# spacemeshos/go-spacemesh

Measured on NVIDIA H100. Metric: POST labels/sec (scrypt N=8192 init), higher is better.
Workload: dtype u32

## Files before the change

go-spacemesh_b200/csrc/capi.cu:

```cuda
#include <algorithm>
#include <chrono>
#include <cstring>
#include <string>
#include <vector>

#include "../../include/b200post.h"
#include "../../include/b200post_verify.h"
#include "../../include/post_compat.h"
#include "engine.h"
#include "host_hash.h"
#include "randomx_engine.h"

using namespace b200post;

namespace {

bool valid_n(uint64_t n) { return n >= 2 && n <= (1ull << 20) && (n & (n - 1)) == 0; }

void fill_nonce(b200post_vrf_nonce *dst, const VrfResult &r) {
    if (!dst) return;
    memset(dst, 0, sizeof *dst);
    dst->found = r.found ? 1 : 0;
    if (r.found) { dst->index = r.index; memcpy(dst->label32, r.label32, 32); }
}
// ... 9 lines not shown
    if (int rc = device_engine(provider, &e)) return rc;
    VrfResult vr;
    const int rc = e->labels_range(commitment, n, start, count, out_host, out_dev, vrf_difficulty, &vr, cancel);
    if (rc == B200POST_OK) fill_nonce(nonce, vr);
    return rc;
}

}

extern "C" {

int b200post_providers(b200post_provider *out, int max) {
    const int n = device_count();
    for (int i = 0; i < n && out && i < max; i++) {
        cudaDeviceProp p;
        if (cudaGetDeviceProperties(&p, i) != cudaSuccess) continue;
        memset(&out[i], 0, sizeof out[i]);
        out[i].id = (uint32_t)i;
        out[i].device_class = B200POST_DEVICE_CLASS_GPU;
        strncpy(out[i].model, p.name, sizeof(out[i].model) - 1);
        out[i].hbm_bytes = p.totalGlobalMem;
        out[i].sm_count = (uint32_t)p.multiProcessorCount;
        out[i].cc_major = (uint32_t)p.major; out[i].cc_minor = (uint32_t)p.minor;
    }
    return n;
}

const char *b200post_last_error(void) { return last_error(); }

int b200post_set_option(const char *key, int64_t value) {
    if (!key) return B200POST_ERR_INVALID_ARGUMENT;
    Options &o = options();
    const std::string k(key);
    if (k == "romix_variant" && value >= 0 && value <= 4) { o.romix_variant = value; return B200POST_OK; }
    if (k == "rotate_mask" && value >= 0 && value <= 1 && romix_mask_supported((int)value)) { o.rotate_mask = value; return B200POST_OK; }
    if (k == "tpb" && (value == 64 || value == 128 || value == 256 || value == 512)) { o.tpb = value; return B200POST_OK; }
    if (k == "dr_unroll" && (value == 1 || value == 4)) { o.dr_unroll = value; return B200POST_OK; }
    if (k == "ctas_per_sm" && value >= 0 && value <= 32) { o.ctas_per_sm = value; return B200POST_OK; }
    if (k == "max_scratch_mib" && value >= 0) { o.max_scratch_mib = value; return B200POST_OK; }
    if (k == "speculate_next" && (value == 0 || value == 1)) { o.speculate_next = value; return B200POST_OK; }
    if (k == "debug_corrupt_next_batch" && (value == 0 || value == 1)) { o.debug_corrupt_next_batch = value; return B200POST_OK; }
    if (k == "debug_corrupt_check_all" && (value == 0 || value == 1)) { o.debug_corrupt_check_all = value; return B200POST_OK; }
    if (k == "lowlat_max_labels" && value >= 0 && value <= (1 << 20)) { o.lowlat_max_labels = value; return B200POST_OK; }
    if (k == "rx_vm_mode" && value >= 0 && value <= 3) { o.rx_vm_mode = value; return B200POST_OK; }
    if (k == "rx_vms_per_sm" && value >= 0 && value <= 4096) { o.rx_vms_per_sm = value; return B200POST_OK; }
    if (k == "debug_skip_phase" && value >= 0 && value <= 3) { o.debug_skip_phase = value; return B200POST_OK; }
    set_error("unknown option or value out of range: " + k);
    return B200POST_ERR_INVALID_ARGUMENT;
}

int64_t b200post_get_option(const char *key) {
    if (!key) return -1;
    Options &o = options();
    const std::string k(key);
    if (k == "romix_variant") return o.romix_variant;
    if (k == "rotate_mask") return o.rotate_mask;
    if (k == "tpb") return o.tpb;
    if (k == "dr_unroll") return o.dr_unroll;
    if (k == "ctas_per_sm") return o.ctas_per_sm;
    if (k == "max_scratch_mib") return o.max_scratch_mib;
    if (k == "speculate_next") return o.speculate_next;
    if (k == "rx_vms_per_sm") return o.rx_vms_per_sm;
    if (k == "rx_vm_mode") return o.rx_vm_mode;
    if (k == "lowlat_max_labels") return o.lowlat_max_labels;
    if (k == "debug_skip_phase") return o.debug_skip_phase;
    return -1;
}
// ... 230 lines not shown
```

go-spacemesh_b200/csrc/engine.cu:

```cuda
#include "engine.h"

#include <algorithm>
#include <cstdio>
#include <cstdlib>
#include <cstring>
#include <map>
#include <memory>
#include <thread>
#include <vector>

#include "../../include/b200post.h"
#include "../../include/b200post_setup.h"
#include "metrics.h"

namespace b200post {

Options &options() { static Options o; return o; }
std::atomic<uint64_t> g_launches{0};

static thread_local std::string t_error;
void set_error(const std::string &msg) { t_error = msg; }
const char *last_error() { return t_error.c_str(); }
int fail(int rc, const std::string &msg) { set_error(msg); return rc; }

// ... 7 lines not shown
    if (copy_stream_.get()) cudaStreamSynchronize(copy_stream_.get());
}

int DeviceEngine::Layer::allocate(uint32_t slots) {
    CUDA_TRY(X.resize((size_t)slots * 8));
    CUDA_TRY(d_out.resize((size_t)slots * 16));
    CUDA_TRY(h_out.resize((size_t)slots * 16));
    CUDA_TRY(d_commit.resize((size_t)slots * 32));
    CUDA_TRY(h_commit.resize((size_t)slots * 32));
    CUDA_TRY(d_idx.resize(slots));
    CUDA_TRY(h_idx.resize(slots));
    CUDA_TRY(d_cidx.resize(slots));
    CUDA_TRY(h_cidx.resize(slots));
    CUDA_TRY(d_exp.resize((size_t)slots * 16));
    CUDA_TRY(h_exp.resize((size_t)slots * 16));
    CUDA_TRY(d_bits.resize(slots / 32));
    CUDA_TRY(d_cnt.resize(1));
    CUDA_TRY(h_cnt.resize(1));
    CUDA_TRY(ev_done.create(cudaEventDisableTiming));
    CUDA_TRY(ev_k3.create(cudaEventDisableTiming));
    CUDA_TRY(ev_in.create(cudaEventDisableTiming));
    CUDA_TRY(ev_exp.create(cudaEventDisableTiming));
    CUDA_TRY(ev_k2a.create(cudaEventDefault));
    CUDA_TRY(ev_k2b.create(cudaEventDefault));
    in_pending = k2_pending = false;
    pend.live = false;
    return B200POST_OK;
}

int DeviceEngine::ensure(uint64_t N, uint64_t want_slots) {
    Options &o = options();
    const int variant = (int)o.romix_variant.load(), mw = (int)o.rotate_mask.load();
    int tpb = (int)o.tpb.load();
    if (variant != ROMIX_PIPELINED && tpb != 128 && tpb != 256) tpb = 128;
    const int dr = (int)o.dr_unroll.load();
    if (!stream_.get()) {
        CUDA_TRY(stream_.create(cudaStreamNonBlocking));
        CUDA_TRY(copy_stream_.create(cudaStreamNonBlocking));
        for (Event &e : ev_call_) CUDA_TRY(e.create(cudaEventDefault));
        CUDA_TRY(d_diff_.resize(8));
        CUDA_TRY(d_range_commit_.resize(8));
        CUDA_TRY(d_running_.resize(1));
        CUDA_TRY(h_running_.resize(1));
    }
    const size_t pads = variant == ROMIX_PIPELINED ? 2 : 1;
    const size_t per_slot = 128 * (size_t)N * pads;
    size_t free_b = 0, total_b = 0;
    CUDA_TRY(cudaMemGetInfo(&free_b, &total_b));
    size_t budget = (size_t)((double)(free_b + v_bytes_) * 0.95);
    const int64_t cap_mib = o.max_scratch_mib.load();
    if (cap_mib > 0) budget = std::min(budget, (size_t)cap_mib << 20);
    const size_t sms = (size_t)prop_.multiProcessorCount;
    const int64_t want_ctas = o.ctas_per_sm.load();
    auto ctas_for = [&](int t) {
        int c = romix_max_ctas_per_sm(variant, mw, t, dr);
        if (want_ctas > 0) c = std::min<int>(c, (int)want_ctas);
        while (c > 0 && per_slot * (size_t)t * sms * (size_t)c > budget) c--;
        return c;
    };
    if (romix_max_ctas_per_sm(variant, mw, tpb, dr) <= 0) { set_error("romix kernel cannot be resident (unsupported variant / mask / tpb combination)"); return B200POST_ERR_INVALID_ARGUMENT; }
    int ctas = ctas_for(tpb);
    if (variant == ROMIX_PIPELINED) {
        for (int t = tpb / 2; t >= 64; t /= 2) {
            const int c = ctas_for(t);
            if ((uint64_t)c * t > (uint64_t)ctas * tpb) { ctas = c; tpb = t; }
        }
    }
    if (ctas == 0) ctas = 1;
    variant_ = variant; mw_ = mw; tpb_ = tpb; dr_unroll_ = dr;
    uint64_t wave = (uint64_t)sms * (uint64_t)ctas * (uint64_t)tpb;
    if (per_slot * wave > budget) {
        wave = budget / per_slot / 32 * 32;
        if (wave == 0) { set_error("not enough HBM for one warp of ROMix scratch"); return B200POST_ERR_OUT_OF_MEMORY; }
    }
    if (wave != wave_slots_) spec_.valid = false;
    wave_slots_ = (uint32_t)wave;

    const uint32_t need = (uint32_t)std::min<uint64_t>(wave, round_up((uint32_t)std::min<uint64_t>(want_slots, wave), 32));
    const size_t need_v = per_slot * (size_t)need;
    if (need_v > v_bytes_ || 128 * (size_t)N * 32 > v_align_) {
        CUDA_TRY(cudaStreamSynchronize(stream_.get()));
        spec_.valid = false;
        V_raw_.reset(); V_ = nullptr; v_bytes_ = 0;
        const size_t align = std::min<size_t>(128 * (size_t)N * 32, (size_t)1 << 32);
        CUDA_TRY(V_raw_.resize(need_v + align));
        V_ = reinterpret_cast<uint4 *>(((uintptr_t)V_raw_.get() + align - 1) / align * align);
        v_bytes_ = need_v;
        v_align_ = align;
    }
    if (need > alloc_slots_) {
        CUDA_TRY(cudaStreamSynchronize(stream_.get()));
        spec_.valid = false;
        alloc_slots_ = 0;
        for (Layer &l : layer_) { int rc = l.allocate(need); if (rc) return rc; }
        CUDA_TRY(d_cta_cand_.resize(pbkdf2_final_ctas(need)));
        alloc_slots_ = need;
    }
    return B200POST_OK;
}

void DeviceEngine::harvest(int buf) {
    Layer &l = layer_[buf];
    if (!l.k2_pending) return;
    float ms = 0;
    if (cudaEventSynchronize(l.ev_k2b.get()) == cudaSuccess &&
        cudaEventElapsedTime(&ms, l.ev_k2a.get(), l.ev_k2b.get()) == cudaSuccess) {
        romix_ms_ += ms; romix_launches_++; romix_labels_ += l.k2_labels;
    }
    l.k2_pending = false;
}

int DeviceEngine::retire(const Job &job, int b) {
    Layer &l = layer_[b];
    if (!l.pend.live) return B200POST_OK;
    CUDA_TRY(cudaEventSynchronize(l.ev_done.get()));
    if (job.out_host) memcpy(job.out_host + l.pend.off * 16, l.h_out.get(), (size_t)l.pend.n * 16);
    if (job.cmp && *l.h_cnt.get()) {
        std::vector<uint32_t> bits(round_up(l.pend.n, 32) / 32);
        CUDA_TRY(cudaMemcpy(bits.data(), l.d_bits.get(), bits.size() * 4, cudaMemcpyDeviceToHost));
        job.cmp->mismatches += *l.h_cnt.get();
        for (size_t w = 0; w < bits.size() && job.cmp->first.size() < CompareResult::kMaxReported; w++)
            for (uint32_t v = bits[w]; v && job.cmp->first.size() < CompareResult::kMaxReported; v &= v - 1)
                job.cmp->first.push_back(l.pend.off + 32 * w + (uint64_t)__builtin_ctz(v));
    }
    l.pend.live = false;
    return B200POST_OK;
}

int DeviceEngine::stage_layer(const Job &job, uint64_t layer, int b, uint32_t n_valid, LabelJob *lj) {
    Layer &l = layer_[b];
    const uint64_t off = layer * (uint64_t)std::min<uint64_t>(wave_slots_, alloc_slots_);
    *lj = LabelJob{d_range_commit_.get(), 0, nullptr, job.start + off, n_valid, nullptr};
    if (job.gather) {
        if (l.in_pending) { CUDA_TRY(cudaEventSynchronize(l.ev_in.get())); l.in_pending = false; }
        memcpy(l.h_idx.get(), job.indices + off, (size_t)n_valid * 8);
        CUDA_TRY(cudaMemcpyAsync(l.d_idx.get(), l.h_idx.get(), (size_t)n_valid * 8, cudaMemcpyHostToDevice, stream_.get()));
        lj->indices = l.d_idx.get();
        lj->start = 0;
        if (job.commit_index) {
            memcpy(l.h_cidx.get(), job.commit_index + off, (size_t)n_valid * 4);
            CUDA_TRY(cudaMemcpyAsync(l.d_cidx.get(), l.h_cidx.get(), (size_t)n_valid * 4, cudaMemcpyHostToDevice, stream_.get()));
            lj->commit = reinterpret_cast<const uint32_t *>(d_ctab_.get());
            lj->commit_index = l.d_cidx.get();
        } else if (job.commitments) {
            memcpy(l.h_commit.get(), job.commitments + off * 32, (size_t)n_valid * 32);
            CUDA_TRY(cudaMemcpyAsync(l.d_commit.get(), l.h_commit.get(), (size_t)n_valid * 32, cudaMemcpyHostToDevice, stream_.get()));
            lj->commit = reinterpret_cast<const uint32_t *>(l.d_commit.get());
            lj->commit_stride = 8;
        }
        CUDA_TRY(cudaEventRecord(l.ev_in.get(), stream_.get()));
        l.in_pending = true;
    }
    CUDA_TRY(launch_pbkdf2_expand(*lj, l.X.get(), alloc_slots_, round_up(n_valid, 32), stream_.get()));
    g_launches += 1;
    return B200POST_OK;
}

int DeviceEngine::finish_layer(const Job &job, uint64_t layer, int b, uint32_t n_valid, const LabelJob &lj) {
    Layer &l = layer_[b];
    const uint64_t off = layer * (uint64_t)std::min<uint64_t>(wave_slots_, alloc_slots_);
    const uint32_t n_slots = round_up(n_valid, 32);
    if (job.expect_host) {
        memcpy(l.h_exp.get(), job.expect_host + off * 16, (size_t)n_valid * 16);
        CUDA_TRY(cudaMemcpyAsync(l.d_exp.get(), l.h_exp.get(), (size_t)n_valid * 16, cudaMemcpyHostToDevice, copy_stream_.get()));
        CUDA_TRY(cudaEventRecord(l.ev_exp.get(), copy_stream_.get()));
        CUDA_TRY(cudaStreamWaitEvent(stream_.get(), l.ev_exp.get(), 0));
        CUDA_TRY(cudaMemsetAsync(l.d_cnt.get(), 0, 4, stream_.get()));
        CUDA_TRY(launch_pbkdf2_final_compare(lj, l.X.get(), alloc_slots_, n_slots, l.d_exp.get(), l.d_bits.get(), l.d_cnt.get(),
                                           job.d_diff, d_cta_cand_.get(), stream_.get()));
    } else if (job.out_hi_dev) {
        CUDA_TRY(launch_pbkdf2_final_wide(lj, l.X.get(), alloc_slots_, n_slots, job.out_dev + off * 16, job.out_hi_dev + off * 16,
                                          stream_.get()));
    } else {
        uint8_t *d_out = job.out_dev ? job.out_dev + off * 16 : l.d_out.get();
        CUDA_TRY(launch_pbkdf2_final(lj, l.X.get(), alloc_slots_, n_slots, d_out, job.d_diff, d_cta_cand_.get(), stream_.get()));
    }
    g_launches += 1;
    if (job.d_diff) {
        CUDA_TRY(launch_vrf_merge(d_cta_cand_.get(), pbkdf2_final_ctas(n_slots), d_running_.get(), stream_.get()));
        g_launches += 1;
    }
    if (job.out_host || job.expect_host) {
        CUDA_TRY(cudaEventRecord(l.ev_k3.get(), stream_.get()));
        CUDA_TRY(cudaStreamWaitEvent(copy_stream_.get(), l.ev_k3.get(), 0));
        if (job.expect_host)
            CUDA_TRY(cudaMemcpyAsync(l.h_cnt.get(), l.d_cnt.get(), 4, cudaMemcpyDeviceToHost, copy_stream_.get()));
        else
            CUDA_TRY(cudaMemcpyAsync(l.h_out.get(), l.d_out.get(), (size_t)n_valid * 16, cudaMemcpyDeviceToHost, copy_stream_.get()));
        CUDA_TRY(cudaEventRecord(l.ev_done.get(), copy_stream_.get()));
    } else {
        CUDA_TRY(cudaEventRecord(l.ev_done.get(), stream_.get()));
    }
    l.pend = Layer::Pending{off, n_valid, true};
    return B200POST_OK;
}

int DeviceEngine::run_job(const Job &job) {
    const uint64_t S = std::min<uint64_t>(wave_slots_, alloc_slots_);
    const uint64_t M = (job.total + S - 1) / S;
    int rc_ = B200POST_OK, status = B200POST_OK;
    auto layer_count = [&](uint64_t m) { return (uint32_t)std::min<uint64_t>(S, job.total - m * S); };
    cudaStream_t st = stream_.get();

    const int64_t lowlat_max = options().lowlat_max_labels.load();
    const bool lowlat = variant_ == ROMIX_PIPELINED && M == 1 && lowlat_max > 0 && job.total <= (uint64_t)lowlat_max &&
                        job.total <= (uint64_t)prop_.multiProcessorCount * 4 * 32;
    if (lowlat || variant_ != ROMIX_PIPELINED) {
        spec_.valid = false;
        for (uint64_t m = 0; m < M; m++) {
            if (job.cancel && *job.cancel) { status = B200POST_ERR_CANCELLED; break; }
            const int b = (int)(m & 1);
            Layer &l = layer_[b];
            if ((rc_ = retire(job, b))) return rc_;
            harvest(b);
            const uint32_t n_valid = layer_count(m);
            LabelJob lj;
            if ((rc_ = stage_layer(job, m, b, n_valid, &lj))) return rc_;
            RomixParams rp;
            rp.V = V_; rp.X = l.X.get(); rp.x_stride = alloc_slots_; rp.N = (uint32_t)job.N;
            CUDA_TRY(cudaEventRecord(l.ev_k2a.get(), st));
            if (lowlat) {
                rp.n_slots = n_valid; rp.flags = 0;
                CUDA_TRY(launch_romix_lowlat(mw_, rp, romix_lowlat_warps(n_valid, prop_.multiProcessorCount), st));
            } else {
                rp.n_slots = round_up(n_valid, 32); rp.flags = (uint32_t)options().debug_skip_phase.load();
                CUDA_TRY(launch_romix(variant_, mw_, tpb_, rp, st));
            }
            CUDA_TRY(cudaEventRecord(l.ev_k2b.get(), st));
            l.k2_pending = true; l.k2_labels = n_valid;
            g_launches += 1;
            if ((rc_ = finish_layer(job, m, b, n_valid, lj))) return rc_;
        }
    } else {
        const bool resume = !job.gather && spec_.valid && spec_.N == job.N && spec_.next_start == job.start &&
                            !memcmp(spec_.commitment, cur_commitment_, 32);
        const int poff = resume ? spec_.parity : 0;
        spec_.valid = false;
        const bool speculate = !job.gather && options().speculate_next.load() != 0 && M >= 4 && job.start + job.total + S > job.start + job.total;
        auto par = [&](uint64_t m) { return (int)((m + (uint64_t)poff) & 1); };
        LabelJob lj[2];
        uint32_t nv[2] = {0, 0};
        bool spec_filled = false;
        for (uint64_t m = 0; m <= M; m++) {
            if (m < M && job.cancel && *job.cancel) { status = B200POST_ERR_CANCELLED; break; }
            const int b = par(m);
            Layer &l = layer_[b];
            harvest(b);
            bool fill = false;
            uint32_t n_fill = 0;
            if (m < M) {
                nv[b] = layer_count(m);
                if (m == 0 && resume) {
                    lj[b] = LabelJob{d_range_commit_.get(), 0, nullptr, job.start, nv[b], nullptr};
                } else {
                    if ((rc_ = stage_layer(job, m, b, nv[b], &lj[b]))) return rc_;
                    fill = true; n_fill = round_up(nv[b], 32);
                }
            } else if (speculate && status == B200POST_OK) {
// ... 291 lines not shown
```

go-spacemesh_b200/csrc/engine.h:

```cpp
#pragma once
#include <cuda_runtime.h>

#include <atomic>
#include <cstdint>
#include <functional>
#include <mutex>
#include <string>
#include <vector>

#include "label_kernels.cuh"
#include "cuda_util.h"

namespace b200post {

struct Options {
    std::atomic<int64_t> romix_variant{ROMIX_PIPELINED};
    std::atomic<int64_t> rotate_mask{0};
    std::atomic<int64_t> tpb{512};
    std::atomic<int64_t> dr_unroll{4};
    std::atomic<int64_t> ctas_per_sm{0};
    std::atomic<int64_t> max_scratch_mib{0};
    std::atomic<int64_t> speculate_next{1};
    std::atomic<int64_t> lowlat_max_labels{4096};
    std::atomic<int64_t> rx_vms_per_sm{0};
    std::atomic<int64_t> rx_vm_mode{1};
    std::atomic<int64_t> debug_corrupt_next_batch{0};
    std::atomic<int64_t> debug_corrupt_check_all{0};
    std::atomic<int64_t> debug_skip_phase{0};
};
Options &options();

extern std::atomic<uint64_t> g_launches;

struct VrfResult { bool found = false; uint64_t index = 0; uint8_t label32[32] = {0}; };
struct CompareResult {
    static constexpr size_t kMaxReported = 64;
    uint64_t mismatches = 0;
    std::vector<uint64_t> first;
};

void set_error(const std::string &msg);
const char *last_error();
int fail(int rc, const std::string &msg);

class DeviceEngine {
public:
    explicit DeviceEngine(int device);
    ~DeviceEngine();
    DeviceEngine(const DeviceEngine &) = delete;
// ... 45 lines not shown
        DeviceBuffer<uint32_t> d_bits, d_cnt;
        PinnedBuffer<uint32_t> h_cnt;
        Event ev_done;
        Event ev_k3;
        Event ev_in;
        Event ev_exp;
        Event ev_k2a, ev_k2b;
        bool in_pending = false, k2_pending = false;
        double k2_labels = 0;
        struct Pending { uint64_t off; uint32_t n; bool live; } pend{0, 0, false};
        int allocate(uint32_t slots);
    };
    int call(Job &job, const std::function<int()> &setup);
    int ensure(uint64_t N, uint64_t want_slots);
    int run_job(const Job &job);
    int range_call(Job &job, const uint8_t commitment[32], const uint8_t *vrf_difficulty);
    int upload_commitment(const uint8_t commitment[32]);
    int stage_layer(const Job &job, uint64_t layer, int b, uint32_t n_valid, LabelJob *lj);
    int finish_layer(const Job &job, uint64_t layer, int b, uint32_t n_valid, const LabelJob &lj);
    int retire(const Job &job, int buf);
    void harvest(int buf);
    void quiesce();

    int dev_;
    cudaDeviceProp prop_{};
    std::mutex mu_;
    Stream stream_;
    Stream copy_stream_;
    DeviceBuffer<uint8_t> V_raw_;
    uint4 *V_ = nullptr;
    size_t v_bytes_ = 0, v_align_ = 0;
    uint32_t alloc_slots_ = 0;
    uint32_t wave_slots_ = 0;
    Layer layer_[2];
    DeviceBuffer<uint32_t> d_range_commit_;
    DeviceBuffer<uint8_t> d_ctab_;
    DeviceBuffer<uint32_t> d_diff_;
    DeviceBuffer<VrfCandidate> d_cta_cand_, d_running_;
    PinnedBuffer<VrfCandidate> h_running_;
    Event ev_call_[2];
    double last_call_ms_ = 0;
    Event ev_timer_[2];
    double romix_ms_ = 0, romix_labels_ = 0;
    uint64_t romix_launches_ = 0;
    struct Speculation {
        bool valid = false;
        uint8_t commitment[32] = {0};
        uint64_t N = 0, next_start = 0;
        int parity = 0;
    } spec_;
    uint8_t cur_commitment_[32] = {0};
    int variant_ = ROMIX_PIPELINED, mw_ = 0, tpb_ = 512, dr_unroll_ = 4;
};

DeviceEngine *engine_for(uint32_t provider);
int device_engine(uint32_t provider, DeviceEngine **e = nullptr);
int device_engines(const uint32_t *providers, int n, std::vector<DeviceEngine *> *out = nullptr);
int device_count();
int provider_devices(int64_t provider_id, std::vector<uint32_t> *devs);
void shutdown_all();

int fan_out(size_t parts, const std::function<int(size_t)> &part);

int label32_at(DeviceEngine *e, const uint8_t commitment[32], uint64_t N, uint64_t index, uint8_t out[32]);

}
// ... 1 lines not shown
```

go-spacemesh_b200/csrc/label_kernels.cu:

```cuda
#include "label_kernels.cuh"

namespace b200post {

__device__ __forceinline__ uint32_t smem_u32(const void *p) { return (uint32_t)__cvta_generic_to_shared(p); }

__device__ __forceinline__ uint4 ld_stream(const uint4 *p) {
    uint4 v;
    asm volatile("ld.global.cs.v4.u32 {%0,%1,%2,%3}, [%4];" : "=r"(v.x), "=r"(v.y), "=r"(v.z), "=r"(v.w) : "l"(p));
    return v;
}
__device__ __forceinline__ void st_stream(uint4 *p, const uint4 &v) {
    asm volatile("st.global.cs.v4.u32 [%0], {%1,%2,%3,%4};" ::"l"(p), "r"(v.x), "r"(v.y), "r"(v.z), "r"(v.w) : "memory");
}
__device__ __forceinline__ void cp_async16(uint32_t dst_smem, const void *src) {
    asm volatile("cp.async.cg.shared.global [%0], [%1], 16;" ::"r"(dst_smem), "l"(src) : "memory");
}
template <int IMM>
__device__ __forceinline__ void cp_async16_lohi(uint32_t dst_smem, uint32_t lo, uint32_t hi) {
    asm volatile("{\n\t.reg .b64 a;\n\tmov.b64 a, {%1, %2};\n\tcp.async.cg.shared.global [%0], [a+%3], 16;\n\t}"
                 ::"r"(dst_smem), "r"(lo), "r"(hi), "n"(IMM) : "memory");
}
template <int IMM>
__device__ __forceinline__ void st_stream_lohi(uint32_t lo, uint32_t hi, const uint4 &v) {
    asm volatile("{\n\t.reg .b64 a;\n\tmov.b64 a, {%0, %1};\n\tst.global.cs.v4.u32 [a+%2], {%3,%4,%5,%6};\n\t}"
// ... 272 lines not shown
    };

    if (do_mix) mix_prefetch();
    for (uint32_t i = 0; i < N; i++) {
        if (do_fill) {
            fill_store();
            blockmix_r1<MW, DR_UNROLL>(lo_f, hi_f);
        }
        if (do_mix) {
            cp_async_wait_all();
            __syncwarp();
            uint32_t vlo[16], vhi[16];
#pragma unroll
            for (int k = 0; k < 8; k++) set_chunk(vlo, vhi, k, lds128(own_m + ((k ^ swz) << 4)));
            __syncwarp();
            blockmix_r1_xor<MW, DR_UNROLL>(lo_m, hi_m, vlo, vhi);
            if (i + 1 < N) mix_prefetch();
        }
    }
#undef MIX_PREFETCH_K
#undef FILL_STORE_K
    if (do_fill) {
#pragma unroll
        for (int k = 0; k < 8; k++) p.Xfill[(size_t)k * p.x_stride + slot] = ROW_CHUNK(lo_f, hi_f, k);
    }
    if (do_mix) {
#pragma unroll
        for (int k = 0; k < 8; k++) p.Xmix[(size_t)k * p.x_stride + slot] = ROW_CHUNK(lo_m, hi_m, k);
    }
    if (p.cta_trace && threadIdx.x == 0) {
        unsigned long long t;
        asm volatile("mov.u64 %0, %%globaltimer;" : "=l"(t));
        p.cta_trace[3 * (size_t)blockIdx.x + 1] = t;
    }
}

constexpr int FINAL_TPB = 128;

__device__ __forceinline__ void warp_argmin(uint32_t (&best)[8], uint64_t &best_i, uint32_t &has) {
#pragma unroll
    for (int off = 16; off > 0; off >>= 1) {
        uint32_t o[8];
#pragma unroll
        for (int k = 0; k < 8; k++) o[k] = __shfl_xor_sync(0xffffffffu, best[k], off);
        const uint64_t oi = __shfl_xor_sync(0xffffffffu, best_i, off);
        const uint32_t oh = __shfl_xor_sync(0xffffffffu, has, off);
        const bool take = oh && (!has || cand_less(o, oi, best, best_i));
        if (take) {
#pragma unroll
            for (int k = 0; k < 8; k++) best[k] = o[k];
            best_i = oi; has = 1;
        }
    }
}

__device__ __forceinline__ void cta_vrf_candidate(bool valid, const uint32_t (&lab)[8], uint64_t index,
                                                  const uint32_t *__restrict__ vrf_be, VrfCandidate *warp_best,
                                                  VrfCandidate *__restrict__ cta_cand) {
    uint32_t diff[8];
#pragma unroll
    for (int k = 0; k < 8; k++) diff[k] = vrf_be[k];
    const bool cand = valid && cand_less(lab, 0, diff, 0);
    if (!__syncthreads_or(cand)) {
        if (threadIdx.x == 0) cta_cand[blockIdx.x].found = 0;
        return;
    }
// ... 181 lines not shown
cudaError_t launch_pbkdf2_final_compare(const LabelJob &job, const uint4 *X, uint32_t x_stride, uint32_t n_slots,
                                        const uint8_t *expect16, uint32_t *mismatch_bits, uint32_t *mismatch_count,
                                        const uint32_t *vrf_difficulty_be, VrfCandidate *cta_cand, cudaStream_t s) {
    if (n_slots == 0) return cudaSuccess;
    pbkdf2_final_compare_kernel<<<pbkdf2_final_ctas(n_slots), FINAL_TPB, 0, s>>>(job, X, x_stride, n_slots, expect16, mismatch_bits,
                                                                                 mismatch_count, vrf_difficulty_be, cta_cand);
    return cudaGetLastError();
}

cudaError_t launch_pbkdf2_final(const LabelJob &job, const uint4 *X, uint32_t x_stride, uint32_t n_slots, uint8_t *out16,
                                const uint32_t *vrf_difficulty_be, VrfCandidate *cta_cand, cudaStream_t s) {
    if (n_slots == 0) return cudaSuccess;
    pbkdf2_final_kernel<<<pbkdf2_final_ctas(n_slots), FINAL_TPB, 0, s>>>(job, X, x_stride, n_slots, out16,
                                                                         vrf_difficulty_be, cta_cand);
    return cudaGetLastError();
}

cudaError_t launch_pbkdf2_final_wide(const LabelJob &job, const uint4 *X, uint32_t x_stride, uint32_t n_slots, uint8_t *out16,
                                     uint8_t *out_hi16, cudaStream_t s) {
    if (n_slots == 0) return cudaSuccess;
    pbkdf2_final_wide_kernel<<<pbkdf2_final_ctas(n_slots), FINAL_TPB, 0, s>>>(job, X, x_stride, n_slots, out16, out_hi16);
    return cudaGetLastError();
}

cudaError_t launch_vrf_merge(const VrfCandidate *cta_cand, uint32_t n_cta, VrfCandidate *running, cudaStream_t s) {
    vrf_merge_kernel<<<1, 256, 0, s>>>(cta_cand, n_cta, running);
    return cudaGetLastError();
}

size_t romix_smem_bytes(int variant, int tpb) {
    const size_t warps = (size_t)tpb / 32;
    if (variant == ROMIX_COALESCED) return warps * 4096;
    if (variant == ROMIX_BULK) return warps * 8192 + warps * 8;
    if (variant == ROMIX_PIPELINED) return warps * 8192;
    return 0;
}

const char *romix_variant_name(int variant) {
    switch (variant) {
        case ROMIX_DIRECT: return "direct";
        case ROMIX_COALESCED: return "coalesced";
        case ROMIX_BULK: return "bulk";
        case ROMIX_NOMEM: return "nomem";
        case ROMIX_PIPELINED: return "pipelined";
    }
    return "?";
}

typedef void (*romix_fn)(const RomixParams);
typedef void (*pipe_fn)(const PipeParams);

#define B200POST_MW_LIST(X) X(0) X(1)

template <int VARIANT, int MW>
static romix_fn pick_tpb(int tpb) {
    switch (tpb) {
        case 128: return romix_kernel<VARIANT, MW, 128>;
        case 256: return romix_kernel<VARIANT, MW, 256>;
    }
    return nullptr;
}
template <int VARIANT>
static romix_fn pick_mw(int mw, int tpb) {
    switch (mw) {
#define X(m) case m: return pick_tpb<VARIANT, m>(tpb);
        B200POST_MW_LIST(X)
#undef X
    }
    return nullptr;
}
static romix_fn pick(int variant, int mw, int tpb) {
    switch (variant) {
        case ROMIX_DIRECT: return pick_mw<ROMIX_DIRECT>(mw, tpb);
        case ROMIX_COALESCED: return pick_mw<ROMIX_COALESCED>(mw, tpb);
        case ROMIX_BULK: return pick_mw<ROMIX_BULK>(mw, tpb);
        case ROMIX_NOMEM: return pick_mw<ROMIX_NOMEM>(mw, tpb);
    }
    return nullptr;
}
template <int MW>
static pipe_fn pick_pipe_tpb(int tpb, int dr_unroll) {
    if (dr_unroll == 4) {
        switch (tpb) {
            case 64: return romix_pipe_kernel<MW, 64, 4>;
            case 128: return romix_pipe_kernel<MW, 128, 4>;
            case 256: return romix_pipe_kernel<MW, 256, 4>;
            case 512: return romix_pipe_kernel<MW, 512, 4>;
        }
    } else {
        switch (tpb) {
            case 64: return romix_pipe_kernel<MW, 64, 1>;
            case 128: return romix_pipe_kernel<MW, 128, 1>;
            case 256: return romix_pipe_kernel<MW, 256, 1>;
            case 512: return romix_pipe_kernel<MW, 512, 1>;
        }
    }
    return nullptr;
}
static pipe_fn pick_pipe(int mw, int tpb, int dr_unroll) {
    switch (mw) {
#define X(m) case m: return pick_pipe_tpb<m>(tpb, dr_unroll);
        B200POST_MW_LIST(X)
#undef X
    }
    return nullptr;
}

bool romix_mask_supported(int mw) {
    switch (mw) {
#define X(m) case m: return true;
        B200POST_MW_LIST(X)
#undef X
    }
    return false;
}

int romix_max_ctas_per_sm(int variant, int rot_mask, int tpb, int dr_unroll) {
    const size_t smem = romix_smem_bytes(variant, tpb);
    int n = 0;
    if (variant == ROMIX_PIPELINED) {
        pipe_fn fn = pick_pipe(rot_mask, tpb, dr_unroll);
        if (!fn) return 0;
        if (smem > 48 * 1024) cudaFuncSetAttribute(fn, cudaFuncAttributeMaxDynamicSharedMemorySize, (int)smem);
        if (cudaOccupancyMaxActiveBlocksPerMultiprocessor(&n, fn, tpb, smem) != cudaSuccess) return 0;
        return n;
    }
    romix_fn fn = pick(variant, rot_mask, tpb);
    if (!fn) return 0;
    if (smem > 48 * 1024) cudaFuncSetAttribute(fn, cudaFuncAttributeMaxDynamicSharedMemorySize, (int)smem);
    if (cudaOccupancyMaxActiveBlocksPerMultiprocessor(&n, fn, tpb, smem) != cudaSuccess) return 0;
    return n;
}

cudaError_t launch_romix(int variant, int rot_mask, int tpb, const RomixParams &p, cudaStream_t s) {
    if (p.n_slots == 0) return cudaSuccess;
    romix_fn fn = pick(variant, rot_mask, tpb);
    if (!fn) return cudaErrorInvalidValue;
    const size_t smem = romix_smem_bytes(variant, tpb);
    if (smem > 48 * 1024) {
        cudaError_t e = cudaFuncSetAttribute(fn, cudaFuncAttributeMaxDynamicSharedMemorySize, (int)smem);
        if (e != cudaSuccess) return e;
    }
    fn<<<(p.n_slots + tpb - 1) / tpb, tpb, smem, s>>>(p);
    return cudaGetLastError();
}

uint32_t romix_lowlat_warps(uint32_t n_slots, int sm_count) {
    const uint32_t full = (uint32_t)sm_count * 4;
    return n_slots < full ? (n_slots ? n_slots : 1) : full;
}
cudaError_t launch_romix_lowlat(int rot_mask, const RomixParams &p, uint32_t n_warps, cudaStream_t s) {
    if (p.n_slots == 0) return cudaSuccess;
    if (n_warps == 0 || (uint64_t)n_warps * 32 < p.n_slots) return cudaErrorInvalidValue;
    if (rot_mask == 1) romix_lowlat_kernel<1><<<n_warps, 32, 0, s>>>(p, n_warps);
    else romix_lowlat_kernel<0><<<n_warps, 32, 0, s>>>(p, n_warps);
    return cudaGetLastError();
}

cudaError_t launch_romix_pipe(int rot_mask, int tpb, int dr_unroll, const PipeParams &p, cudaStream_t s) {
    const uint32_t n = p.n_fill > p.n_mix ? p.n_fill : p.n_mix;
    if (n == 0) return cudaSuccess;
    pipe_fn fn = pick_pipe(rot_mask, tpb, dr_unroll);
    if (!fn) return cudaErrorInvalidValue;
    const size_t smem = romix_smem_bytes(ROMIX_PIPELINED, tpb);
    if (smem > 48 * 1024) {
        cudaError_t e = cudaFuncSetAttribute(fn, cudaFuncAttributeMaxDynamicSharedMemorySize, (int)smem);
        if (e != cudaSuccess) return e;
    }
    fn<<<(n + tpb - 1) / tpb, tpb, smem, s>>>(p);
    return cudaGetLastError();
}

}
```

go-spacemesh_b200/csrc/label_kernels.cuh:

```cuda
#pragma once
#include <cuda_runtime.h>
#include <cstdint>

#include "post_device.cuh"

namespace b200post {

enum RomixVariant : int {
    ROMIX_DIRECT = 0,
    ROMIX_COALESCED = 1,
    ROMIX_BULK = 2,
    ROMIX_NOMEM = 3,
    ROMIX_PIPELINED = 4,
};

struct RomixParams {
    uint4 *V;
    uint4 *X;
    uint32_t x_stride;
    uint32_t N;
    uint32_t n_slots;
    uint32_t flags;
};

struct PipeParams {
    uint4 *V;
    uint4 *Xfill;
    uint4 *Xmix;
    uint32_t x_stride;
    uint32_t N;
    uint32_t n_fill, n_mix;
    uint32_t fill_parity;
    unsigned long long *cta_trace;
};

struct LabelJob {
    const uint32_t *commit;
    uint32_t commit_stride;
    const uint64_t *indices;
    uint64_t start;
    uint32_t n_valid;
    const uint32_t *commit_index;
};

struct VrfCandidate {
    uint32_t label_be[8];
    uint64_t index;
    uint32_t found, pad;
};

cudaError_t launch_pbkdf2_expand(const LabelJob &job, uint4 *X, uint32_t x_stride, uint32_t n_slots, cudaStream_t s);
cudaError_t launch_romix(int variant, int rot_mask, int tpb, const RomixParams &p, cudaStream_t s);
cudaError_t launch_romix_pipe(int rot_mask, int tpb, int dr_unroll, const PipeParams &p, cudaStream_t s);
uint32_t romix_lowlat_warps(uint32_t n_slots, int sm_count);
cudaError_t launch_romix_lowlat(int rot_mask, const RomixParams &p, uint32_t n_warps, cudaStream_t s);
// ... 19 lines not shown
```

go-spacemesh_b200/csrc/post_device.cuh:

```cuda
#pragma once
#include <cstdint>

#if defined(__CUDACC__)
#define PD_HD __host__ __device__ __forceinline__
#define PD_D __device__ __forceinline__
#else
#define PD_HD inline
#define PD_D inline
#endif

namespace b200post {

PD_HD uint32_t rotl(uint32_t x, int k) {
#if defined(__CUDA_ARCH__)
    return __funnelshift_l(x, x, k);
#else
    return (x << k) | (x >> (32 - k));
#endif
}
PD_HD uint32_t bswap32(uint32_t x) {
#if defined(__CUDA_ARCH__)
    return __byte_perm(x, 0, 0x0123);
#else
    return (x >> 24) | ((x >> 8) & 0xff00u) | ((x << 8) & 0xff0000u) | (x << 24);
// ... 47 lines not shown

template <int ROT, int DR_UNROLL = 4>
PD_HD void blockmix_r1(uint32_t (&lo)[16], uint32_t (&hi)[16]) {
#pragma unroll
    for (int i = 0; i < 16; i++) lo[i] ^= hi[i];
    chacha20_8<ROT, DR_UNROLL>(lo);
#pragma unroll
    for (int i = 0; i < 16; i++) hi[i] ^= lo[i];
    chacha20_8<ROT, DR_UNROLL>(hi);
}
template <int ROT, int DR_UNROLL = 4>
PD_HD void blockmix_r1_xor(uint32_t (&lo)[16], uint32_t (&hi)[16], const uint32_t (&vlo)[16],
                           const uint32_t (&vhi)[16]) {
#pragma unroll
    for (int i = 0; i < 16; i++) { hi[i] ^= vhi[i]; lo[i] = lo[i] ^ vlo[i] ^ hi[i]; }
    chacha20_8<ROT, DR_UNROLL>(lo);
#pragma unroll
    for (int i = 0; i < 16; i++) hi[i] ^= lo[i];
    chacha20_8<ROT, DR_UNROLL>(hi);
}

template <int ROT, int DR_UNROLL>
PD_HD void blockmix_r1_dual(uint32_t (&lo_f)[16], uint32_t (&hi_f)[16], uint32_t (&lo_m)[16], uint32_t (&hi_m)[16],
                            const uint32_t (&vlo)[16], const uint32_t (&vhi)[16]) {
#pragma unroll
    for (int i = 0; i < 16; i++) {
        lo_f[i] ^= hi_f[i];
        hi_m[i] ^= vhi[i]; lo_m[i] = lo_m[i] ^ vlo[i] ^ hi_m[i];
    }
    chacha20_8_x2<ROT, DR_UNROLL>(lo_f, lo_m);
#pragma unroll
    for (int i = 0; i < 16; i++) { hi_f[i] ^= lo_f[i]; hi_m[i] ^= lo_m[i]; }
    chacha20_8_x2<ROT, DR_UNROLL>(hi_f, hi_m);
}

#define PD_KECCAK_RC_TABLE \
    0x0000000000000001ull, 0x0000000000008082ull, 0x800000000000808aull, 0x8000000080008000ull, 0x000000000000808bull, \
    0x0000000080000001ull, 0x8000000080008081ull, 0x8000000000008009ull, 0x000000000000008aull, 0x0000000000000088ull, \
    0x0000000080008009ull, 0x000000008000000aull, 0x000000008000808bull, 0x800000000000008bull, 0x8000000000008089ull, \
    0x8000000000008003ull, 0x8000000000008002ull, 0x8000000000000080ull, 0x000000000000800aull, 0x800000008000000aull, \
    0x8000000080008081ull, 0x8000000000008080ull, 0x0000000080000001ull, 0x8000000080008008ull
static const uint64_t h_KeccakRC[24] = {PD_KECCAK_RC_TABLE};
#if defined(__CUDACC__)
static __device__ __constant__ uint64_t c_KeccakRC[24] = {PD_KECCAK_RC_TABLE};
#endif
PD_HD uint64_t keccak_rc(int i) {
#if defined(__CUDA_ARCH__)
    return c_KeccakRC[i];
#else
    return h_KeccakRC[i];
#endif
}
PD_HD uint64_t rotl64(uint64_t x, int k) { return (x << k) | (x >> (64 - k)); }

PD_HD void keccak_f1600(uint64_t (&s)[25]) {
#pragma unroll 1
    for (int round = 0; round < 24; round++) {
        const uint64_t c0 = s[0] ^ s[5] ^ s[10] ^ s[15] ^ s[20], c1 = s[1] ^ s[6] ^ s[11] ^ s[16] ^ s[21],
                       c2 = s[2] ^ s[7] ^ s[12] ^ s[17] ^ s[22], c3 = s[3] ^ s[8] ^ s[13] ^ s[18] ^ s[23],
                       c4 = s[4] ^ s[9] ^ s[14] ^ s[19] ^ s[24];
        const uint64_t d0 = c4 ^ rotl64(c1, 1), d1 = c0 ^ rotl64(c2, 1), d2 = c1 ^ rotl64(c3, 1),
                       d3 = c2 ^ rotl64(c4, 1), d4 = c3 ^ rotl64(c0, 1);
#pragma unroll
        for (int y = 0; y < 25; y += 5) { s[y] ^= d0; s[y + 1] ^= d1; s[y + 2] ^= d2; s[y + 3] ^= d3; s[y + 4] ^= d4; }
        uint64_t t = s[1], u;
#define PD_RP(j, r) u = s[j]; s[j] = rotl64(t, r); t = u;
// ... 133 lines not shown
```

Before: 1.235 million.

## Add phased ROMix kernel processing two labels per thread as default

Adds a new ROMix variant in which each thread carries two independent scrypt states (slot and slot+T). Their fill-phase blockmixes are interleaved, and in the read phase each state's random-row cp.async fetch overlaps the other state's mix. The intent is to hide HBM latency with instruction-level parallelism instead of warp-level occupancy. The engine now sizes a layer at twice the wave, sets the new variant as the default, and drops the speculative pipelined path. The cost is doubled registers per thread, which may reduce occupancy.

```diff
diff --git a/go-spacemesh_b200/csrc/capi.cu b/go-spacemesh_b200/csrc/capi.cu
--- a/go-spacemesh_b200/csrc/capi.cu
+++ b/go-spacemesh_b200/csrc/capi.cu
@@ -65,7 +65,7 @@
     if (!key) return B200POST_ERR_INVALID_ARGUMENT;
     Options &o = options();
     const std::string k(key);
-    if (k == "romix_variant" && value >= 0 && value <= 4) { o.romix_variant = value; return B200POST_OK; }
+    if (k == "romix_variant" && value >= 0 && value <= 5) { o.romix_variant = value; return B200POST_OK; }
     if (k == "rotate_mask" && value >= 0 && value <= 1 && romix_mask_supported((int)value)) { o.rotate_mask = value; return B200POST_OK; }
     if (k == "tpb" && (value == 64 || value == 128 || value == 256 || value == 512)) { o.tpb = value; return B200POST_OK; }
     if (k == "dr_unroll" && (value == 1 || value == 4)) { o.dr_unroll = value; return B200POST_OK; }
diff --git a/go-spacemesh_b200/csrc/engine.cu b/go-spacemesh_b200/csrc/engine.cu
--- a/go-spacemesh_b200/csrc/engine.cu
+++ b/go-spacemesh_b200/csrc/engine.cu
@@ -63,7 +63,8 @@
     Options &o = options();
     const int variant = (int)o.romix_variant.load(), mw = (int)o.rotate_mask.load();
     int tpb = (int)o.tpb.load();
-    if (variant != ROMIX_PIPELINED && tpb != 128 && tpb != 256) tpb = 128;
+    const bool two_pads = variant == ROMIX_PIPELINED || variant == ROMIX_PHASED;
+    if (!two_pads && tpb != 128 && tpb != 256) tpb = 128;
     const int dr = (int)o.dr_unroll.load();
     if (!stream_.get()) {
         CUDA_TRY(stream_.create(cudaStreamNonBlocking));
@@ -74,7 +75,7 @@
         CUDA_TRY(d_running_.resize(1));
         CUDA_TRY(h_running_.resize(1));
     }
-    const size_t pads = variant == ROMIX_PIPELINED ? 2 : 1;
+    const size_t pads = two_pads ? 2 : 1;
     const size_t per_slot = 128 * (size_t)N * pads;
     size_t free_b = 0, total_b = 0;
     CUDA_TRY(cudaMemGetInfo(&free_b, &total_b));
@@ -91,7 +92,7 @@
     };
     if (romix_max_ctas_per_sm(variant, mw, tpb, dr) <= 0) { set_error("romix kernel cannot be resident (unsupported variant / mask / tpb combination)"); return B200POST_ERR_INVALID_ARGUMENT; }
     int ctas = ctas_for(tpb);
-    if (variant == ROMIX_PIPELINED) {
+    if (two_pads) {
         for (int t = tpb / 2; t >= 64; t /= 2) {
             const int c = ctas_for(t);
             if ((uint64_t)c * t > (uint64_t)ctas * tpb) { ctas = c; tpb = t; }
@@ -106,9 +107,11 @@
     }
     if (wave != wave_slots_) spec_.valid = false;
     wave_slots_ = (uint32_t)wave;
-
-    const uint32_t need = (uint32_t)std::min<uint64_t>(wave, round_up((uint32_t)std::min<uint64_t>(want_slots, wave), 32));
-    const size_t need_v = per_slot * (size_t)need;
+    const uint64_t layer = variant == ROMIX_PHASED ? 2 * wave : wave;
+    layer_labels_ = (uint32_t)layer;
+
+    const uint32_t need = (uint32_t)std::min<uint64_t>(layer, round_up((uint32_t)std::min<uint64_t>(want_slots, layer), 32));
+    const size_t need_v = per_slot * (size_t)std::min<uint64_t>(need, wave);
     if (need_v > v_bytes_ || 128 * (size_t)N * 32 > v_align_) {
         CUDA_TRY(cudaStreamSynchronize(stream_.get()));
         spec_.valid = false;
@@ -160,7 +163,7 @@
 
 int DeviceEngine::stage_layer(const Job &job, uint64_t layer, int b, uint32_t n_valid, LabelJob *lj) {
     Layer &l = layer_[b];
-    const uint64_t off = layer * (uint64_t)std::min<uint64_t>(wave_slots_, alloc_slots_);
+    const uint64_t off = layer * (uint64_t)std::min<uint64_t>(layer_labels_, alloc_slots_);
     *lj = LabelJob{d_range_commit_.get(), 0, nullptr, job.start + off, n_valid, nullptr};
     if (job.gather) {
         if (l.in_pending) { CUDA_TRY(cudaEventSynchronize(l.ev_in.get())); l.in_pending = false; }
@@ -189,7 +192,7 @@
 
 int DeviceEngine::finish_layer(const Job &job, uint64_t layer, int b, uint32_t n_valid, const LabelJob &lj) {
     Layer &l = layer_[b];
-    const uint64_t off = layer * (uint64_t)std::min<uint64_t>(wave_slots_, alloc_slots_);
+    const uint64_t off = layer * (uint64_t)std::min<uint64_t>(layer_labels_, alloc_slots_);
     const uint32_t n_slots = round_up(n_valid, 32);
     if (job.expect_host) {
         memcpy(l.h_exp.get(), job.expect_host + off * 16, (size_t)n_valid * 16);
@@ -227,14 +230,14 @@
 }
 
 int DeviceEngine::run_job(const Job &job) {
-    const uint64_t S = std::min<uint64_t>(wave_slots_, alloc_slots_);
+    const uint64_t S = std::min<uint64_t>(layer_labels_, alloc_slots_);
     const uint64_t M = (job.total + S - 1) / S;
     int rc_ = B200POST_OK, status = B200POST_OK;
     auto layer_count = [&](uint64_t m) { return (uint32_t)std::min<uint64_t>(S, job.total - m * S); };
     cudaStream_t st = stream_.get();
 
     const int64_t lowlat_max = options().lowlat_max_labels.load();
-    const bool lowlat = variant_ == ROMIX_PIPELINED && M == 1 && lowlat_max > 0 && job.total <= (uint64_t)lowlat_max &&
+    const bool lowlat = (variant_ == ROMIX_PIPELINED || variant_ == ROMIX_PHASED) && M == 1 && lowlat_max > 0 && job.total <= (uint64_t)lowlat_max &&
                         job.total <= (uint64_t)prop_.multiProcessorCount * 4 * 32;
     if (lowlat || variant_ != ROMIX_PIPELINED) {
         spec_.valid = false;
@@ -255,6 +258,7 @@
                 CUDA_TRY(launch_romix_lowlat(mw_, rp, romix_lowlat_warps(n_valid, prop_.multiProcessorCount), st));
             } else {
                 rp.n_slots = round_up(n_valid, 32); rp.flags = (uint32_t)options().debug_skip_phase.load();
+                rp.pair_offset = wave_slots_;
                 CUDA_TRY(launch_romix(variant_, mw_, tpb_, rp, st));
             }
             CUDA_TRY(cudaEventRecord(l.ev_k2b.get(), st));
diff --git a/go-spacemesh_b200/csrc/engine.h b/go-spacemesh_b200/csrc/engine.h
--- a/go-spacemesh_b200/csrc/engine.h
+++ b/go-spacemesh_b200/csrc/engine.h
@@ -14,7 +14,7 @@
 namespace b200post {
 
 struct Options {
-    std::atomic<int64_t> romix_variant{ROMIX_PIPELINED};
+    std::atomic<int64_t> romix_variant{ROMIX_PHASED};
     std::atomic<int64_t> rotate_mask{0};
     std::atomic<int64_t> tpb{512};
     std::atomic<int64_t> dr_unroll{4};
@@ -126,6 +126,7 @@
     size_t v_bytes_ = 0, v_align_ = 0;
     uint32_t alloc_slots_ = 0;
     uint32_t wave_slots_ = 0;
+    uint32_t layer_labels_ = 0;
     Layer layer_[2];
     DeviceBuffer<uint32_t> d_range_commit_;
     DeviceBuffer<uint8_t> d_ctab_;
diff --git a/go-spacemesh_b200/csrc/label_kernels.cu b/go-spacemesh_b200/csrc/label_kernels.cu
--- a/go-spacemesh_b200/csrc/label_kernels.cu
+++ b/go-spacemesh_b200/csrc/label_kernels.cu
@@ -328,6 +328,119 @@
         unsigned long long t;
         asm volatile("mov.u64 %0, %%globaltimer;" : "=l"(t));
         p.cta_trace[3 * (size_t)blockIdx.x + 1] = t;
+    }
+}
+
+template <int MW, int TPB>
+__global__ void __launch_bounds__(TPB) romix_phased_kernel(const RomixParams p) {
+    constexpr int DR = 4;
+    extern __shared__ __align__(128) uint8_t smem_raw[];
+    const uint32_t T = p.pair_offset;
+    const uint32_t slot = blockIdx.x * TPB + threadIdx.x;
+    if (slot >= T || slot >= p.n_slots) return;
+    const bool has_b = slot + T < p.n_slots;
+    const uint32_t lane = threadIdx.x & 31, warp_in_cta = threadIdx.x >> 5;
+    const uint32_t N = p.N, mask = N - 1;
+    const uint32_t tile_a = smem_u32(smem_raw) + warp_in_cta * 8192, tile_b = tile_a + 4096;
+    const uint32_t own_a = tile_a + lane * 128, own_b = tile_b + lane * 128;
+    const uint32_t swz = lane & 7, tr_row = lane >> 3, tr_c = lane & 7;
+    const uint32_t tile_a_tr = tile_a + tr_row * 128 + (tr_c << 4), tile_b_tr = tile_b + tr_row * 128 + (tr_c << 4);
+    const size_t warp = slot >> 5;
+    const uint64_t va64 = (uint64_t)(p.V + (warp * 2) * (size_t)N * 256 + lane);
+    const uint64_t vb64 = (uint64_t)(p.V + (warp * 2 + 1) * (size_t)N * 256 + lane);
+    const uint32_t va_lo = (uint32_t)va64, va_hi = (uint32_t)(va64 >> 32);
+    const uint32_t vb_lo = (uint32_t)vb64, vb_hi = (uint32_t)(vb64 >> 32);
+    uint32_t src_lane[8];
+#pragma unroll
+    for (int k = 0; k < 8; k++) src_lane[k] = k * 4 + tr_row;
+
+    uint32_t lo_a[16], hi_a[16], lo_b[16], hi_b[16];
+#pragma unroll
+    for (int k = 0; k < 8; k++) set_chunk(lo_a, hi_a, k, p.X[(size_t)k * p.x_stride + slot]);
+    if (has_b) {
+#pragma unroll
+        for (int k = 0; k < 8; k++) set_chunk(lo_b, hi_b, k, p.X[(size_t)k * p.x_stride + slot + T]);
+    }
+
+#define ROW_TO_TILE(own, lo, hi) \
+    _Pragma("unroll") for (int k = 0; k < 8; k++) sts128(own + ((k ^ swz) << 4), ROW_CHUNK(lo, hi, k));
+#define TILE_TO_HBM_K(tile_tr, cur, vhi, k) st_stream_lohi<(k) * 512>(cur, vhi, lds128(tile_tr + (k) * 512));
+#define TILE_TO_HBM(tile_tr, cur, vhi)                                                                          \
+    TILE_TO_HBM_K(tile_tr, cur, vhi, 0) TILE_TO_HBM_K(tile_tr, cur, vhi, 1) TILE_TO_HBM_K(tile_tr, cur, vhi, 2) \
+    TILE_TO_HBM_K(tile_tr, cur, vhi, 3) TILE_TO_HBM_K(tile_tr, cur, vhi, 4) TILE_TO_HBM_K(tile_tr, cur, vhi, 5) \
+    TILE_TO_HBM_K(tile_tr, cur, vhi, 6) TILE_TO_HBM_K(tile_tr, cur, vhi, 7)
+#define ROW_REQUEST_K(tile_tr, j, vlo, vhi, k) \
+    cp_async16_lohi<(k) * 512>(tile_tr + (k) * 512, mad_u32(__shfl_sync(0xffffffffu, j, src_lane[k]), 4096u, vlo), vhi);
+#define ROW_REQUEST(tile_tr, hi, vlo, vhi)                                                                             \
+    {                                                                                                                  \
+        const uint32_t j = hi[0] & mask;                                                                               \
+        ROW_REQUEST_K(tile_tr, j, vlo, vhi, 0) ROW_REQUEST_K(tile_tr, j, vlo, vhi, 1) ROW_REQUEST_K(tile_tr, j, vlo, vhi, 2) \
+        ROW_REQUEST_K(tile_tr, j, vlo, vhi, 3) ROW_REQUEST_K(tile_tr, j, vlo, vhi, 4) ROW_REQUEST_K(tile_tr, j, vlo, vhi, 5) \
+        ROW_REQUEST_K(tile_tr, j, vlo, vhi, 6) ROW_REQUEST_K(tile_tr, j, vlo, vhi, 7)                                  \
+        cp_async_commit();                                                                                             \
+    }
+#define MIX_FROM_TILE(own, lo, hi)                                                                       \
+    {                                                                                                    \
+        uint32_t vlo[16], vhi[16];                                                                       \
+        _Pragma("unroll") for (int k = 0; k < 8; k++) set_chunk(vlo, vhi, k, lds128(own + ((k ^ swz) << 4))); \
+        __syncwarp();                                                                                    \
+        blockmix_r1_xor<MW, DR>(lo, hi, vlo, vhi);                                                       \
+    }
+
+    uint32_t va_cur = va_lo, vb_cur = vb_lo;
+    if (has_b) {
+        for (uint32_t i = 0; i < N; i++) {
+            ROW_TO_TILE(own_a, lo_a, hi_a)
+            ROW_TO_TILE(own_b, lo_b, hi_b)
+            __syncwarp();
+            TILE_TO_HBM(tile_a_tr, va_cur, va_hi)
+            TILE_TO_HBM(tile_b_tr, vb_cur, vb_hi)
+            __syncwarp();
+            va_cur = mad_u32(1u, 4096u, va_cur); vb_cur = mad_u32(1u, 4096u, vb_cur);
+            blockmix_r1_x2<MW, DR>(lo_a, hi_a, lo_b, hi_b);
+        }
+        ROW_REQUEST(tile_b_tr, hi_b, vb_lo, vb_hi)
+        for (uint32_t i = 0; i < N; i++) {
+            ROW_REQUEST(tile_a_tr, hi_a, va_lo, va_hi)
+            asm volatile("cp.async.wait_group 1;" ::: "memory");
+            __syncwarp();
+            MIX_FROM_TILE(own_b, lo_b, hi_b)
+            if (i + 1 < N) {
+                ROW_REQUEST(tile_b_tr, hi_b, vb_lo, vb_hi)
+                asm volatile("cp.async.wait_group 1;" ::: "memory");
+            } else {
+                cp_async_wait_all();
+            }
+            __syncwarp();
+            MIX_FROM_TILE(own_a, lo_a, hi_a)
+        }
+    } else {
+        for (uint32_t i = 0; i < N; i++) {
+            ROW_TO_TILE(own_a, lo_a, hi_a)
+            __syncwarp();
+            TILE_TO_HBM(tile_a_tr, va_cur, va_hi)
+            __syncwarp();
+            va_cur = mad_u32(1u, 4096u, va_cur);
+            blockmix_r1<MW, DR>(lo_a, hi_a);
+        }
+        for (uint32_t i = 0; i < N; i++) {
+            ROW_REQUEST(tile_a_tr, hi_a, va_lo, va_hi)
+            cp_async_wait_all();
+            __syncwarp();
+            MIX_FROM_TILE(own_a, lo_a, hi_a)
+        }
+    }
+#undef ROW_TO_TILE
+#undef TILE_TO_HBM_K
+#undef TILE_TO_HBM
+#undef ROW_REQUEST_K
+#undef ROW_REQUEST
+#undef MIX_FROM_TILE
+#pragma unroll
+    for (int k = 0; k < 8; k++) p.X[(size_t)k * p.x_stride + slot] = ROW_CHUNK(lo_a, hi_a, k);
+    if (has_b) {
+#pragma unroll
+        for (int k = 0; k < 8; k++) p.X[(size_t)k * p.x_stride + slot + T] = ROW_CHUNK(lo_b, hi_b, k);
     }
 }
 
@@ -575,7 +688,7 @@
     const size_t warps = (size_t)tpb / 32;
     if (variant == ROMIX_COALESCED) return warps * 4096;
     if (variant == ROMIX_BULK) return warps * 8192 + warps * 8;
-    if (variant == ROMIX_PIPELINED) return warps * 8192;
+    if (variant == ROMIX_PIPELINED || variant == ROMIX_PHASED) return warps * 8192;
     return 0;
 }
 
@@ -586,6 +699,7 @@
         case ROMIX_BULK: return "bulk";
         case ROMIX_NOMEM: return "nomem";
         case ROMIX_PIPELINED: return "pipelined";
+        case ROMIX_PHASED: return "phased";
     }
     return "?";
 }
@@ -643,6 +757,25 @@
 static pipe_fn pick_pipe(int mw, int tpb, int dr_unroll) {
     switch (mw) {
 #define X(m) case m: return pick_pipe_tpb<m>(tpb, dr_unroll);
+        B200POST_MW_LIST(X)
+#undef X
+    }
+    return nullptr;
+}
+
+template <int MW>
+static romix_fn pick_phased_tpb(int tpb) {
+    switch (tpb) {
+        case 64: return romix_phased_kernel<MW, 64>;
+        case 128: return romix_phased_kernel<MW, 128>;
+        case 256: return romix_phased_kernel<MW, 256>;
+        case 512: return romix_phased_kernel<MW, 512>;
+    }
+    return nullptr;
+}
+static romix_fn pick_phased(int mw, int tpb) {
+    switch (mw) {
+#define X(m) case m: return pick_phased_tpb<m>(tpb);
         B200POST_MW_LIST(X)
 #undef X
     }
@@ -668,7 +801,7 @@
         if (cudaOccupancyMaxActiveBlocksPerMultiprocessor(&n, fn, tpb, smem) != cudaSuccess) return 0;
         return n;
     }
-    romix_fn fn = pick(variant, rot_mask, tpb);
+    romix_fn fn = variant == ROMIX_PHASED ? pick_phased(rot_mask, tpb) : pick(variant, rot_mask, tpb);
     if (!fn) return 0;
     if (smem > 48 * 1024) cudaFuncSetAttribute(fn, cudaFuncAttributeMaxDynamicSharedMemorySize, (int)smem);
     if (cudaOccupancyMaxActiveBlocksPerMultiprocessor(&n, fn, tpb, smem) != cudaSuccess) return 0;
@@ -677,14 +810,17 @@
 
 cudaError_t launch_romix(int variant, int rot_mask, int tpb, const RomixParams &p, cudaStream_t s) {
     if (p.n_slots == 0) return cudaSuccess;
-    romix_fn fn = pick(variant, rot_mask, tpb);
+    const bool phased = variant == ROMIX_PHASED;
+    romix_fn fn = phased ? pick_phased(rot_mask, tpb) : pick(variant, rot_mask, tpb);
     if (!fn) return cudaErrorInvalidValue;
     const size_t smem = romix_smem_bytes(variant, tpb);
     if (smem > 48 * 1024) {
         cudaError_t e = cudaFuncSetAttribute(fn, cudaFuncAttributeMaxDynamicSharedMemorySize, (int)smem);
         if (e != cudaSuccess) return e;
     }
-    fn<<<(p.n_slots + tpb - 1) / tpb, tpb, smem, s>>>(p);
+    if (phased && (p.pair_offset % 32 || 2 * (uint64_t)p.pair_offset < p.n_slots)) return cudaErrorInvalidValue;
+    const uint32_t threads = phased && p.pair_offset < p.n_slots ? p.pair_offset : p.n_slots;
+    fn<<<(threads + tpb - 1) / tpb, tpb, smem, s>>>(p);
     return cudaGetLastError();
 }
 
diff --git a/go-spacemesh_b200/csrc/label_kernels.cuh b/go-spacemesh_b200/csrc/label_kernels.cuh
--- a/go-spacemesh_b200/csrc/label_kernels.cuh
+++ b/go-spacemesh_b200/csrc/label_kernels.cuh
@@ -12,6 +12,7 @@
     ROMIX_BULK = 2,
     ROMIX_NOMEM = 3,
     ROMIX_PIPELINED = 4,
+    ROMIX_PHASED = 5,
 };
 
 struct RomixParams {
@@ -21,6 +22,7 @@
     uint32_t N;
     uint32_t n_slots;
     uint32_t flags;
+    uint32_t pair_offset;
 };
 
 struct PipeParams {
diff --git a/go-spacemesh_b200/csrc/post_device.cuh b/go-spacemesh_b200/csrc/post_device.cuh
--- a/go-spacemesh_b200/csrc/post_device.cuh
+++ b/go-spacemesh_b200/csrc/post_device.cuh
@@ -103,6 +103,16 @@
 #pragma unroll
     for (int i = 0; i < 16; i++) { hi_f[i] ^= lo_f[i]; hi_m[i] ^= lo_m[i]; }
     chacha20_8_x2<ROT, DR_UNROLL>(hi_f, hi_m);
+}
+
+template <int ROT, int DR_UNROLL>
+PD_HD void blockmix_r1_x2(uint32_t (&lo_a)[16], uint32_t (&hi_a)[16], uint32_t (&lo_b)[16], uint32_t (&hi_b)[16]) {
+#pragma unroll
+    for (int i = 0; i < 16; i++) { lo_a[i] ^= hi_a[i]; lo_b[i] ^= hi_b[i]; }
+    chacha20_8_x2<ROT, DR_UNROLL>(lo_a, lo_b);
+#pragma unroll
+    for (int i = 0; i < 16; i++) { hi_a[i] ^= lo_a[i]; hi_b[i] ^= lo_b[i]; }
+    chacha20_8_x2<ROT, DR_UNROLL>(hi_a, hi_b);
 }
 
 #define PD_KECCAK_RC_TABLE \
```

Result: faster. 1.350 million (median of 6 runs) (+9.3%).
